# cocowy1/Cost-Volume-Aggregation-in-Stereo-Matching-Revisited

Hardware: AMD Instinct MI355X
Metric: cost-volumes/sec (fwd+bwd) at 544x960 D=192 (higher is better)
Workload: dtype f32

## Files before the change

### cost-volume-aggregation-in-stereo-matching-revisited_amd/csrc/conv3d_c1.hip

```cpp
#include "dca_common.h"
#include "dca_tiles.h"
#include "../../include/dca_hip.h"

namespace {
constexpr int TD = 4, TH = 8, TW = 32, CK = 4;
constexpr int ID = TD + 2, IH = TH + 2, IWP = 40;

struct C1Args {
  const float* x;
  const float* w;
  const float* dy;
  float* out;
  int N, C, D, H, W;
  int nTD, nTH, nTW, ntiles;
  int vec;
};

__device__ __forceinline__ void stage_tile(const float* __restrict__ src, float* lds, int n, int C, int c0, int nch,
                                           int D, int H, int W, int d0, int h0, int w0, int vec, int tid) {
  const int rows = nch * ID * IH;
  if (vec) {
    for (int it = tid; it < rows * 8; it += 256) {
      const int row = it >> 3, q = it & 7;
      const int c = row / (ID * IH), rem = row % (ID * IH), id = rem / IH, ih = rem % IH;
// ... 17 lines not shown
      const int row = it / 34, j = it % 34;
      const int c = row / (ID * IH), rem = row % (ID * IH), id = rem / IH, ih = rem % IH;
      const int ci = c0 + c, d = d0 - 1 + id, h = h0 - 1 + ih, wi = w0 - 1 + j;
      float v = 0.f;
      if (ci < C && (unsigned)d < (unsigned)D && (unsigned)h < (unsigned)H && (unsigned)wi < (unsigned)W)
        v = src[((((long)n * C + ci) * D + d) * H + h) * W + wi];
      lds[row * IWP + 3 + j] = v;
    }
  }
}

__device__ __forceinline__ void tile_coords(const C1Args& a, int tile, int& n, int& d0, int& h0, int& w0) {
  dca_tile_decode<TD, TH, TW>(tile, a.nTD, a.nTH, a.nTW, n, d0, h0, w0);
}

__global__ __launch_bounds__(256) void c1_bwd_data_kernel(C1Args a) {
  __shared__ __attribute__((aligned(16))) float dy_lds[ID * IH * IWP];
  extern __shared__ __attribute__((aligned(16))) float w_lds[];
  const int tid = threadIdx.x, wq = tid & 7, row = tid >> 3, dl = row >> 3, hl = row & 7;
  int n, d0, h0, w0;
  tile_coords(a, xcd_remap(blockIdx.x, gridDim.x), n, d0, h0, w0);
  stage_tile(a.dy, dy_lds, n, 1, 0, 1, a.D, a.H, a.W, d0, h0, w0, a.vec, tid);
  for (int i = tid; i < a.C * 27; i += 256) {
    const int c = i / 27, t = i % 27;
    w_lds[(c * 9 + t / 3) * 4 + t % 3] = a.w[c * 27 + 26 - t];
  }
  __syncthreads();
  float g[9][6];
#pragma unroll
  for (int r9 = 0; r9 < 9; ++r9) {
    const float* p = dy_lds + ((dl + r9 / 3) * IH + hl + r9 % 3) * IWP + 4 * wq;
    const float4 v = *(const float4*)(p + 4);
    g[r9][0] = p[3]; g[r9][1] = v.x; g[r9][2] = v.y; g[r9][3] = v.z; g[r9][4] = v.w; g[r9][5] = p[8];
  }
  const int d = d0 + dl, h = h0 + hl, w = w0 + 4 * wq;
  const bool ok = d < a.D && h < a.H && w < a.W;
  for (int c = 0; c < a.C; ++c) {
    float acc[4] = {0.f, 0.f, 0.f, 0.f};
#pragma unroll
    for (int r9 = 0; r9 < 9; ++r9) {
      const float4 wv = *(const float4*)(w_lds + (c * 9 + r9) * 4);
#pragma unroll
      for (int j = 0; j < 4; ++j)
        acc[j] = fmaf(wv.z, g[r9][j + 2], fmaf(wv.y, g[r9][j + 1], fmaf(wv.x, g[r9][j], acc[j])));
    }
    if (ok) {
      float* o = a.out + ((((long)n * a.C + c) * a.D + d) * a.H + h) * a.W + w;
      if (a.vec) {
        *(float4*)o = make_float4(acc[0], acc[1], acc[2], acc[3]);
      } else {
#pragma unroll
        for (int j = 0; j < 4; ++j)
          if (w + j < a.W) o[j] = acc[j];
      }
    }
  }
}

__global__ __launch_bounds__(256) void c1_gather_kernel(const float* __restrict__ T, float* __restrict__ y, int D, int H,
                                                        int W) {
  const long DHW = (long)D * H * W;
  const long n = blockIdx.y;
  const float* p = T + n * 27 * DHW;
  const long end = min(DHW, ((long)blockIdx.x + 1) * 1024);
  for (long idx = (long)blockIdx.x * 1024 + threadIdx.x; idx < end; idx += 256) {
    const int w = idx % W;
    const int t = (int)(idx / W);
    const int h = t % H, d = t / H;
// ... 55 lines not shown
      for (int j = 0; j < 4; ++j) v[j] = dca_bload1(dr, base + 4 * j, okr & (int)((unsigned)(w0 + j) < (unsigned)W));
    }
    *(float4*)(out + 4 * (long)q) = make_float4(v[0], v[1], v[2], v[3]);
  }
}

int fill_args(C1Args& a, int N, int C, int D, int H, int W, const void* p0, const void* p1, const void* p2) {
  a.N = N; a.C = C; a.D = D; a.H = H; a.W = W;
  a.nTD = cdiv(D, TD); a.nTH = cdiv(H, TH); a.nTW = cdiv(W, TW);
  const long nt = (long)N * a.nTD * a.nTH * a.nTW;
  if (nt >= (1L << 31)) return 1;
  a.ntiles = (int)nt;
  a.vec = (W % 4 == 0) && ((((uintptr_t)p0 | (uintptr_t)p1 | (uintptr_t)p2) & 15) == 0);
  return 0;
}
}

extern "C" int dca_conv3d_c1_bwd_data(const float* dy, const float* w, float* dx, int N, int C, int D, int H, int W,
                                      hipStream_t stream) {
  DCA_REQUIRE(dy && w && dx && N > 0 && C > 0 && C <= 256 && D > 0 && H > 0 && W > 0);
  C1Args a;
  a.x = nullptr; a.w = w; a.dy = dy; a.out = dx;
  DCA_REQUIRE(fill_args(a, N, C, D, H, W, dy, dx, nullptr) == 0);
  hipLaunchKernelGGL(c1_bwd_data_kernel, dim3(a.ntiles), dim3(256), (size_t)C * 36 * 4, stream, a);
  return dca_launch_status();
}

extern "C" int dca_conv3d_c1_gather(const float* T, float* y, int N, int D, int H, int W, hipStream_t stream) {
  DCA_REQUIRE(T && y && N > 0 && D > 0 && H > 0 && W > 0);
  DCA_REQUIRE(9L * D * H * W * 4 < 0x7ffffff0L && N <= 65535);
// ... 15 lines not shown
```

### cost-volume-aggregation-in-stereo-matching-revisited_amd/csrc/pointwise.hip

```cpp
#include "dca_frag.h"
#include "../../include/dca_hip.h"

__global__ __launch_bounds__(256) void bn_stats_kernel(const float* __restrict__ x, double* __restrict__ part, int N,
                                                       int C, long S, int nchunk, long chunk_len, int vec) {
  const int c = blockIdx.x, ch = blockIdx.y, tid = threadIdx.x;
  const long s0 = ch * chunk_len, s1 = min(S, s0 + chunk_len);
  const float K = x[(long)c * S];
  if (ch == 0 && tid == 0) part[(long)C * nchunk * 2 + c] = (double)K;
  float s = 0.f, ss = 0.f;
  for (int n = 0; n < N; ++n) {
    const float* p = x + ((long)n * C + c) * S;
    if (vec) {
      for (long i = s0 + 4 * tid; i < s1; i += 1024) {
        float4 v = *(const float4*)(p + i);
        v.x -= K; v.y -= K; v.z -= K; v.w -= K;
        s += (v.x + v.y) + (v.z + v.w);
        ss += (v.x * v.x + v.y * v.y) + (v.z * v.z + v.w * v.w);
      }
    } else {
      for (long i = s0 + tid; i < s1; i += 256) {
        const float v = p[i] - K;
        s += v;
        ss += v * v;
      }
// ... 96 lines not shown
  const float mean = (float)(kref + ms), var = (float)v;
  if (running_mean) {
    const double unb = n > 1.0 ? v * n / (n - 1.0) : v;
    running_mean[c] = (1.f - momentum) * running_mean[c] + momentum * mean;
    running_var[c] = (1.f - momentum) * running_var[c] + momentum * (float)unb;
  }
  const float invstd = 1.0f / sqrtf(var + eps);
  stats[c] = mean;
  stats[C + c] = invstd;
  stats[2 * C + c] = g * invstd;
  stats[3 * C + c] = b - mean * g * invstd;
  if (zexps) zexps[c] = ze;
}


__device__ __forceinline__ float bn_affine(float y, float sc, float sh) { return __fmaf_rn(y, sc, sh); }
__device__ __forceinline__ float bn_skip(float y, float sc, float sh) { return act_apply(bn_affine(y, sc, sh), 1.f); }
__device__ __forceinline__ void bn_bwd_acc(float g, float y, float mean, float invstd, float& a0, float& a1) {
#pragma clang fp contract(off)
  a0 += g;
  a1 += g * (y - mean) * invstd;
}

__global__ __launch_bounds__(256) void bn_apply_kernel(const float* __restrict__ y, const float* __restrict__ stats,
                                                       const float* __restrict__ res_pre, const float* __restrict__ res_post,
                                                       float* __restrict__ z, int N, int C, long S, long chunk_len,
                                                       float slope, int vec, unsigned* __restrict__ zmax,
                                                       unsigned* __restrict__ ymax) {
  const int c = blockIdx.y, ch = blockIdx.x, tid = threadIdx.x;
  const long s0 = ch * chunk_len, s1 = min(S, s0 + chunk_len);
  const float mean = stats[c], sc = stats[2 * C + c], sh = stats[3 * C + c];
  float am = 0.f, ym = 0.f;
  for (int n = N - 1; n >= 0; --n) {
    const long base = ((long)n * C + c) * S;
    if (vec) {
      for (long i = s0 + 4 * tid; i < s1; i += 1024) {
        float4 v = *(const float4*)(y + base + i);
// ... 9 lines not shown
      for (long i = s0 + tid; i < s1; i += 256) {
        const float yv = y[base + i];
        ym = fmaxf(ym, fabsf(yv - mean));
        float v = bn_affine(yv, sc, sh);
        if (res_pre) v += res_pre[base + i];
        v = act_apply(v, slope);
        if (res_post) v += res_post[base + i];
        z[base + i] = v;
        am = fmaxf(am, fabsf(v));
      }
    }
  }
  if (zmax) dca_cmax_put(am, zmax + (long)c * DCA_AMAX_CSLOTS + ch);
  if (ymax) dca_cmax_put(ym, ymax + (long)c * DCA_AMAX_CSLOTS + ch);
}

__device__ __forceinline__ void px2_split(float v, int e, unsigned short& h, unsigned short& l) {
  _Float16 hh, ll;
  x2_split(v, e, hh, ll);
  h = __builtin_bit_cast(unsigned short, hh);
  l = __builtin_bit_cast(unsigned short, ll);
}
typedef unsigned short u16x8 __attribute__((ext_vector_type(8)));

template <bool SKIP>
__global__ __launch_bounds__(256) void bn_apply_pack_kernel(const float* __restrict__ y, const float* __restrict__ stats,
                                                            const int* __restrict__ zexps, char* __restrict__ zp, int N,
                                                            int C, long S, long chunk_len, float slope,
                                                            unsigned* __restrict__ ymax, const float* __restrict__ res_pre,
                                                            const float* __restrict__ res_post, float* __restrict__ zf,
                                                            unsigned* __restrict__ zmax, const float* __restrict__ y_r,
                                                            const float* __restrict__ stats_r) {
  const int cg = blockIdx.y, ch = blockIdx.x, tid = threadIdx.x;
  const long s0 = ch * chunk_len, s1 = min(S, s0 + chunk_len);
  float mean[8], sc[8], sh[8], scr[8], shr[8], ym[8], zm[8];
  int ex[8];
#pragma unroll
  for (int j = 0; j < 8; ++j) {
// ... 910 lines not shown

extern "C" int dca_bn_backward_reduce(const float* dz, const float* y, const float* stats, double* part, float* dgb, int N,
                                      int C, long S, float slope, int training, hipStream_t stream) {
  DCA_REQUIRE(dz && y && stats && part && dgb && N > 0 && C > 0 && S > 0 && C <= 65535);
  int nchunk; long len;
  chunking(S, C, &nchunk, &len);
  const int vec = (S % 4 == 0) && ((((uintptr_t)dz | (uintptr_t)y) & 15) == 0);
  hipLaunchKernelGGL(bn_bwd_reduce_kernel, dim3(C, nchunk), dim3(256), 0, stream, dz, y, (const float*)nullptr, stats, part,
                     N, C, S, nchunk, len, slope, vec, (unsigned*)nullptr, (const float*)nullptr, (const float*)nullptr,
                     (double*)nullptr);
  hipLaunchKernelGGL(bn_bwd_finalize_kernel, dim3(C), dim3(64), 0, stream, part, nchunk, (double)N * (double)S, dgb, C,
                     stats, training, (const unsigned*)nullptr, (const unsigned*)nullptr, 0, (int*)nullptr);
  return dca_launch_status();
}

extern "C" int dca_bn_backward_pack(const float* dz, const float* y, const float* stats, double* part, float* dgb, void* dyp,
                                    int* dyexps, unsigned* gmax, const unsigned* ymax, int ymax_slots, int N, int C, long S,
                                    float slope, int training, hipStream_t stream) {
  DCA_REQUIRE(dz && y && stats && part && dgb && dyp && dyexps && gmax && N > 0 && C > 0 && C % 8 == 0 && S > 0 && C <= 65535);
  DCA_REQUIRE((ymax == nullptr || (ymax_slots > 0 && ymax_slots <= DCA_AMAX_CSLOTS)) && ((((uintptr_t)dyp) & 15) == 0));
  int nchunk; long len;
  chunking(S, C, &nchunk, &len);
  const uintptr_t al = (uintptr_t)dz | (uintptr_t)y;
  const int vec = (S % 4 == 0) && ((al & 15) == 0);
  hipLaunchKernelGGL(bn_bwd_reduce_kernel, dim3(C, nchunk), dim3(256), 0, stream, dz, y, (const float*)nullptr, stats, part,
                     N, C, S, nchunk, len, slope, vec, gmax, (const float*)nullptr, (const float*)nullptr, (double*)nullptr);
  hipLaunchKernelGGL(bn_bwd_finalize_kernel, dim3(C), dim3(64), 0, stream, part, nchunk, (double)N * (double)S, dgb, C,
                     stats, training, (const unsigned*)gmax, ymax, ymax_slots, dyexps);
  int pchunk; long plen;
  chunking(S, C / 8, &pchunk, &plen);
// ... 66 lines not shown
```

### cost-volume-aggregation-in-stereo-matching-revisited_amd/models/augment/cva.py

```python
import torch
import torch.nn as nn

from .._bootstrap import ensure as _ensure
from ..submodule import ConvBn3d, ConvBnReLU3d, conv3d_plain, convbn_3d
from .semantic_level import SemanticLevelContext

ops = _ensure().ops


class _DeconvBn3d(nn.Sequential):

    def __init__(self, cin, cout):
        super().__init__(nn.ConvTranspose3d(cin, cout, 3, padding=1, output_padding=1, stride=2, bias=False),
                         nn.BatchNorm3d(cout))

    def forward(self, x, slope=1.0, res_pre=None, res_post=None, pack_out=False):
        return ops.convbn3d(x, self[0], self[1], slope, res_pre, res_post, pack_out=pack_out)


class Multi_Aggregation(nn.Module):

    def __init__(self, in_channels):
        super().__init__()
        self.conv1 = ConvBnReLU3d(in_channels, in_channels * 2, 3, 2, 1)
# ... 15 lines not shown
                         nn.ReLU(inplace=True))

    def forward(self, x):
        return self[1](ops.avg_pool3d_k3s2p1(x), slope=0.0)


class _Classify(nn.Sequential):

    def __init__(self, c):
        super().__init__(ConvBn3d(c, c, 3, 1, 1), nn.ReLU(inplace=True),
                         nn.Conv3d(c, 1, kernel_size=3, padding=1, stride=1, bias=False))

    def forward(self, x, alias=False):
        if alias:
            h, xa = self[0](x, slope=0.0, alias=True)
            return conv3d_plain(h, self[2]), xa
        h = self[0](x, slope=0.0)
        if h.dtype != torch.float32:
            return ops.conv3d_c1_lp(h, self[2].weight)
        return conv3d_plain(h, self[2])


class cva(nn.Module):

    def __init__(self, max_disp, in_channel, downsample=True):
        super().__init__()
        self.max_disp = max_disp
        self.channel = in_channel
        if downsample:
            self.downsample = _Downsample()
        self.slc_net = SemanticLevelContext(feats_channels=self.channel, transform_channels=self.channel,
                                            concat_input=True)
        self.classify = _Classify(self.channel)
        self.fuse = nn.Sequential(ConvBn3d(64, 32, 1, 1, 0))
        self.cost_agg = Multi_Aggregation(self.channel)
# ... 40 lines not shown
```

### cost-volume-aggregation-in-stereo-matching-revisited_amd/models/submodule.py

```python
import torch
import torch.nn as nn
import torch.nn.functional as F

from ._bootstrap import ensure as _ensure

ops = _ensure().ops


def disparity_regression(x, maxdisp):
    assert len(x.shape) == 4
    assert x.shape[1] == maxdisp
    return ops.regression(x)


def build_concat_volume(refimg_fea, targetimg_fea, maxdisp):
    return ops.concat_volume(refimg_fea, targetimg_fea, maxdisp)


def groupwise_correlation(fea1, fea2, num_groups):
    B, C, H, W = fea1.shape
    assert C % num_groups == 0
    cost = ops.gwc_volume(fea1, fea2, 1, num_groups)[:, :, 0]
    assert cost.shape == (B, num_groups, H, W)
    return cost
# ... 17 lines not shown
        assert (kernel_size, pad) in ((3, 1), (1, 0)) and stride in (1, 2)

    def forward(self, x, slope=1.0, res_pre=None, res_post=None, x2=None, alias=False, pack_out=False):
        return ops.convbn3d(x, self[0], self[1], slope, res_pre, res_post, x2, alias, pack_out)


class ConvBnReLU3d(nn.Sequential):

    def __init__(self, in_channels, out_channels, kernel_size, stride, pad):
        super().__init__(ConvBn3d(in_channels, out_channels, kernel_size, stride, pad), nn.ReLU(inplace=True))

    def forward(self, x):
        return self[0](x, slope=0.0)


def conv3d_plain(x, conv):
    return ops.conv3d(x, conv.weight, conv.stride[0], False)


def convbn(in_channels, out_channels, kernel_size, stride, pad, dilation):
    return nn.Sequential(nn.Conv2d(in_channels, out_channels, kernel_size=kernel_size, stride=stride,
                                   padding=dilation if dilation > 1 else pad, dilation=dilation, bias=False),
                         nn.BatchNorm2d(out_channels))


class BasicBlock(nn.Module):
    expansion = 1

    def __init__(self, inplanes, planes, stride, downsample, pad, dilation):
        super().__init__()
        self.conv1 = nn.Sequential(convbn(inplanes, planes, 3, stride, pad, dilation), nn.ReLU(inplace=True))
        self.conv2 = convbn(planes, planes, 3, 1, pad, dilation)
# ... 99 lines not shown
```

### cost-volume-aggregation-in-stereo-matching-revisited_amd/ops.py

```python
from __future__ import annotations

import ctypes
import os
import threading

import torch

from ._call import _C, _L, _chk, _ptr, _raw_device, _raw_stream, _req, _req_no_grad, _stream, _vp


def _opt(t, name):
    return None if t is None else _req(t, name)


class _GwcVolume(torch.autograd.Function):
    @staticmethod
    def forward(ctx, ref, tgt, maxdisp, num_groups):
        ref, tgt = _req(ref, "build_gwc_volume"), _req(tgt, "build_gwc_volume")
        B, C, H, W = ref.shape
        vol = torch.empty((B, num_groups, maxdisp, H, W), device=ref.device, dtype=torch.float32)
        with torch.cuda.device_of(ref):
            _chk(_L().dca_gwc_volume_fwd(_ptr(ref), _ptr(tgt), _ptr(vol), B, C, H, W, maxdisp, num_groups, _stream()),
                 "dca_gwc_volume_fwd")
        ctx.save_for_backward(ref, tgt)
# ... 208 lines not shown

def _round_up(a, m):
    return (a + m - 1) // m * m


_CONV_MODE = os.environ.get("DCA_CONV", "x2")
CONV_X3 = _CONV_MODE != "fp32"
CONV_X2 = _CONV_MODE == "x2"
WGRAD_S2_X2 = os.environ.get("DCA_WGRAD_S2", "x2") != "fp32"
DECONV_X3 = os.environ.get("DCA_DECONV", "x3") != "fp32"
C1_WGRAD_FUSED = os.environ.get("DCA_C1_WGRAD", "fused") != "expand"
CONV_S2_X2 = os.environ.get("DCA_CONV_S2", "x2") != "fp32"
BN_FUSE = os.environ.get("DCA_BN_FUSE", "1") != "0"
C1_BWD_FUSE = os.environ.get("DCA_C1_BWD", "fused") != "split"
SKIP_FOLD = os.environ.get("DCA_SKIP_FOLD", "1") != "0"
_X3_MIN_WORKGROUPS = 1


AMAX_STATS = {"tagged": 0, "computed": 0, "packed": 0}
CSLOTS = _C["DCA_AMAX_CSLOTS"]
AMAX_EMIT = os.environ.get("DCA_AMAX_EMIT", "1") != "0"
PACK = os.environ.get("DCA_PACK", "1") != "0"


def _cslots(C, device):
    if not AMAX_EMIT:
        return None
    return torch.empty((C * CSLOTS,), device=device, dtype=torch.int32)


# ... 163 lines not shown
    y, stats, dgb, slope, training = tag
    if y.shape != dz.shape or y.shape[0] != x.shape[0] or y.shape[2:] != x.shape[2:]:
        raise RuntimeError("conv3d.backward: the BatchNorm's gradient does not belong to this convolution")
    N, C1 = x.shape[0], x.shape[1]
    C2 = 0 if x2 is None else x2.shape[1]
    S = x[0, 0].numel()
    lib = _L()
    part = torch.empty((lib.dca_conv1_bwd_fused_workspace(N, S, int(x2 is not None)),), device=x.device, dtype=torch.float32)
    gx = torch.empty_like(x)
    gx2 = None if x2 is None else torch.empty_like(x2)
    gw = torch.empty_like(weight)
    _chk(lib.dca_conv1_bwd_fused(_ptr(dz), _ptr(y), _ptr(stats), _ptr(dgb), float(slope), int(training), _ptr(x), _ptr(x2),
                                 _ptr(weight), _ptr(part), _ptr(gx), _ptr(gx2), _ptr(gw), C1 + C2, 1, N, C1, C2,
                                 weight.shape[0], S, _stream()), "dca_conv1_bwd_fused")
    return gx, gx2, gw


class _SkipBn:
    __slots__ = ("y", "part", "bn", "into")

    def __init__(self, y, part, bn, into):
        self.y, self.part, self.bn, self.into = y, part, bn, into


def _skip_fold_route(x, conv_b, bn_b, slope_b, bn_out):
    if not (SKIP_FOLD and PACK and CONV_X2 and bn_out is not None and torch.is_grad_enabled() and _lp_dtype() is None):
        return "apply"
    C = bn_b.num_features
    if not (bn_b.training and bn_out.training) or bn_out.num_features != C or C % 8 or float(slope_b) != 1.0:
        return "apply"
# ... 215 lines not shown
             "dca_conv3d_wgrad_x3")
    elif family == "s2x2":
        xex, yex = _exps_of(x), _exps_of(dy)
        part = workspace(lib.dca_conv3d_wgrad_s2_x2_workspace(N, Cx, Cy, Di, Hi, Wi))
        _chk(lib.dca_conv3d_wgrad_s2_x2(_ptr(x), _ptr(xex), _ptr(dy), _ptr(yex), _ptr(part), dst, N, Cx, Cy, Di, Hi, Wi,
                                        s_cy, s_cx, _stream()), "dca_conv3d_wgrad_s2_x2")
    else:
        part = workspace(lib.dca_conv3d_wgrad_workspace(N, Cx, Cy, Do, Ho, Wo, ksize, stride))
        _chk(lib.dca_conv3d_wgrad(_ptr(x), _ptr(dy), _ptr(part), dst, N, Cx, Cy, Di, Hi, Wi, Do, Ho, Wo, ksize, stride,
                                  s_cy, s_cx, _stream()), "dca_conv3d_wgrad")


class _Conv3dC1(torch.autograd.Function):

    @staticmethod
    def forward(ctx, x, weight):
        x, weight = _req(x, "conv3d"), _req(weight, "conv3d.weight")
        N, C, D, H, W = x.shape
        with torch.cuda.device_of(x):
            T = _conv_sliced(x, None, weight, C, 27, 1, 1, 0, 1, 1, False)
            y = torch.empty((N, 1, D, H, W), device=x.device, dtype=torch.float32)
            _chk(_L().dca_conv3d_c1_gather(_ptr(T), _ptr(y), N, D, H, W, _stream()), "dca_conv3d_c1_gather")
        ctx.save_for_backward(x, weight)
        return y

    @staticmethod
    def backward(ctx, dy):
        x, weight = ctx.saved_tensors
        dy = _req(dy, "conv3d.backward")
        N, C, D, H, W = x.shape
        gx = gw = None
        lib = _L()
        with torch.cuda.device_of(x):
            if ctx.needs_input_grad[0]:
                gx = torch.empty_like(x)
                _chk(lib.dca_conv3d_c1_bwd_data(_ptr(dy), _ptr(weight), _ptr(gx), N, C, D, H, W, _stream()),
                     "dca_conv3d_c1_bwd_data")
            if ctx.needs_input_grad[1]:
                gw = torch.empty_like(weight)
                if (C1_WGRAD_FUSED and W % 4 == 0 and x.data_ptr() % 16 == 0 and dy.data_ptr() % 16 == 0
                        and x.numel() * 4 < 0x7ffffff0):
                    nws = lib.dca_conv3d_wgrad_workspace(N, C, 27, D, H, W, 1, 1)
                    part = torch.empty((nws,), device=x.device, dtype=torch.float32)
                    _chk(lib.dca_conv3d_c1_wgrad(_ptr(x), _ptr(dy), _ptr(part), _ptr(gw), N, C, D, H, W, _stream()),
                         "dca_conv3d_c1_wgrad")
                else:
                    G = torch.empty((N, 27, D, H, W), device=x.device, dtype=torch.float32)
                    _chk(lib.dca_conv3d_c1_expand(_ptr(dy), _ptr(G), N, D, H, W, _stream()), "dca_conv3d_c1_expand")
                    _wgrad(x, G, gw, 0, C, 27, 1, 1, 1, 27)
        return gx, gw


class _Conv3d(torch.autograd.Function):

    @staticmethod
    def forward(ctx, x, x2, weight, stride, transposed, want_stats=False, alias=False, packed_dy=False, lazy_dy=False):
        x, weight = _req(x, "conv3d", packed_ok=True), _req(weight, "conv3d.weight")
        x2 = _opt(x2, "conv3d.x2")
        if _is_packed(x) and alias:
            raise RuntimeError("conv3d: alias output of a packed px2 operand")
        ctx.save_for_backward(x, x2, weight)
        ctx.meta = (stride, transposed)
        ctx.alias = bool(alias)
        ctx.set_materialize_grads(False)
        ctx.x_px2 = getattr(x, "_dca_px2", None)
# ... 140 lines not shown
          and conv_b.kernel_size[0] == 1 and conv_b.weight.shape[0] in (32, 64) and x.dtype == torch.float32
          and not isinstance(conv_a, torch.nn.ConvTranspose3d) and all(d % 2 == 0 for d in x.shape[2:]))
    if not ok:
        return convbn3d(x, conv_a, bn_a, slope_a, pack_out=pack_a), convbn3d(x, conv_b, bn_b, slope_b)
    stats = bool(BN_FUSE and bn_a.training and bn_b.training)
    fold = _skip_fold_route(x, conv_b, bn_b, slope_b, skip_into) == "fold"
    lazy = fold or _c1_bwd_route(x, None, conv_b.weight) == "fused"
    ya, pa, yb, pb = _ConvPair.apply(x, conv_a.weight, conv_b.weight, stats, lazy)
    za = bn_act(ya, bn_a, slope_a, stats_part=pa if pa.numel() else None, pack_out=pack_a)
    if fold:
        return za, _SkipBn(yb, pb if pb.numel() else None, bn_b, skip_into)
    zb = bn_act(yb, bn_b, slope_b, stats_part=pb if pb.numel() else None, lazy_dy=lazy)
    return za, zb


def conv3d(x, weight, stride=1, transposed=False, x2=None):
    if _k3s1(weight, stride, transposed, x2, head=True) and weight.shape[1] in (32, 64):
        return _Conv3dC1.apply(x, weight)
    return _Conv3d.apply(x, x2, weight, int(stride), bool(transposed))


def conv3d_fused_inference(x, weight, stride, transposed, scale, shift, slope, res_pre=None, res_post=None, x2=None):
    x, weight = _req(x, "conv3d"), _req(weight, "conv3d.weight")
    with torch.cuda.device_of(x):
        return _conv_forward_impl(x, _opt(x2, "x2"), weight, int(stride), bool(transposed), _opt(scale, "scale"),
                                  _opt(shift, "shift"), slope, _opt(res_pre, "res_pre"), _opt(res_post, "res_post"),
                                  emit_amax=CONV_X2 and AMAX_EMIT)


def bn_stats_vector(y, gamma, beta, running_mean, running_var, training, momentum, eps, part=None, zexps=None,
                    rpre=None, rpost=None):
    rps, rpn = rpre if rpre is not None else (None, 0)
# ... 65 lines not shown
                _tag_px2(zp, zexps)
                if pack_z == 2:
                    _tag_twin(z, zp)
            else:
                _chk(lib.dca_bn_apply(_ptr(y), _ptr(stats), _ptr(res_pre), _ptr(res_post), _ptr(z), N, C, S, float(slope),
                                      _ptr(zmax), _ptr(ymax), _stream()), "dca_bn_apply")
                ymax_slots = lib.dca_bn_num_chunks(C, S)
        ctx.save_for_backward(y, stats, res_pre if slope != 1.0 else None, ymax)
        ctx.meta = (training, slope, res_pre is not None, res_post is not None, pack_dy, ymax_slots)
        return z if pack_z == 1 else _tag_cmax(z, zmax, ymax_slots)

    @staticmethod
    def backward(ctx, dz):
        y, stats, res_pre, ymax = ctx.saved_tensors
        training, slope, has_pre, has_post, pack_dy, ymax_slots = ctx.meta
        dz = _req(dz, "batch_norm.backward")
        N, C = y.shape[0], y.shape[1]
        S = y[0, 0].numel()
        lib = _L()
        with torch.cuda.device_of(y):
            nchunk = lib.dca_bn_num_chunks(C, S)
            part = torch.empty((C * nchunk * 2,), device=y.device, dtype=torch.float64)
            dgb = torch.empty((4 * C,), device=y.device, dtype=torch.float32)
            g_out = None
            if ctx.lazy_dy:
                _chk(lib.dca_bn_backward_reduce(_ptr(dz), _ptr(y), _ptr(stats), _ptr(part), _ptr(dgb), N, C, S, float(slope),
                                                int(training), _stream()), "dca_bn_backward_reduce")
                dy = dz.view_as(dz)
                dy._dca_lazy = (y, stats, dgb, slope, training)
            elif pack_dy:
# ... 6 lines not shown
                _tag_px2(dy, dyexps)
            else:
                dy = torch.empty_like(y)
                want_g = has_pre and slope != 1.0 and ctx.needs_input_grad[9]
                g_out = torch.empty_like(y) if want_g else None
                dm = _cslots(C, y.device) if CONV_X2 else None
                _chk(lib.dca_bn_backward(_ptr(dz), _ptr(y), _ptr(res_pre), _ptr(stats), _ptr(part), _ptr(dgb), _ptr(dy),
                                         _ptr(g_out), N, C, S, float(slope), int(training), _ptr(dm), _stream()),
                     "dca_bn_backward")
                _tag_cmax(dy, dm, nchunk)
        g_pre = None
        if has_pre and ctx.needs_input_grad[9]:
            g_pre = g_out if g_out is not None else dz
        g_post = dz if (has_post and ctx.needs_input_grad[10]) else None
        return dy, dgb[:C], dgb[C:2 * C], None, None, None, None, None, None, g_pre, g_post, None, None, None, None, None


class _BnSkipAct(torch.autograd.Function):

    @staticmethod
    def forward(ctx, y, gamma, beta, running_mean, running_var, momentum, eps, part, y_r, gamma_r, beta_r, running_mean_r,
                running_var_r, momentum_r, eps_r, part_r, slope, res_post, zmax):
        y, y_r = _req(y, "batch_norm"), _req(y_r, "batch_norm.skip")
        res_post = _opt(res_post, "res_post")
        if y_r.shape != y.shape:
            raise RuntimeError("batch_norm: the skip branch does not have the output's shape")
        N, C = y.shape[0], y.shape[1]
        S = y[0, 0].numel()
        lib = _L()
        with torch.cuda.device_of(y):
# ... 736 lines not shown
```

### include/dca_hip.h

```cpp
#ifndef DCA_HIP_H
#define DCA_HIP_H

#include <hip/hip_runtime_api.h>

#ifdef __cplusplus
extern "C" {
#endif

#define DCA_ABI_VERSION 21
int dca_abi_version(void);

#define DCA_BF16 1
#define DCA_FP16 2

int dca_gwc_volume_fwd(const float* ref, const float* tgt, float* vol, int B, int C, int H, int W, int maxdisp,
                       int num_groups, hipStream_t stream);
int dca_gwc_volume_bwd(const float* gvol, const float* ref, const float* tgt, float* gref, float* gtgt, int B, int C,
                       int H, int W, int maxdisp, int num_groups, hipStream_t stream);
long dca_gwc_volume_bwd_rows(int B, int C, int H, int W, int maxdisp, int num_groups);
int dca_concat_volume_fwd(const float* ref, const float* tgt, float* vol, int B, int C, int H, int W, int maxdisp,
                          hipStream_t stream);
int dca_concat_volume_bwd(const float* gvol, float* gref, float* gtgt, int B, int C, int H, int W, int maxdisp,
                          hipStream_t stream);

// ... 105 lines not shown
                    int* zexps, const unsigned* rpre_slots, int rpre_n, const unsigned* rpost_slots, int rpost_n, int C,
                    hipStream_t stream);
int dca_bn_apply(const float* y, const float* stats, const float* res_pre, const float* res_post, float* z, int N,
                 int C, long S, float slope, unsigned* zmax, unsigned* ymax, hipStream_t stream);
int dca_bn_apply_pack(const float* y, const float* stats, const int* zexps, void* zp, int N, int C, long S, float slope,
                      unsigned* ymax, const float* res_pre, const float* res_post, float* zf, unsigned* zmax,
                      hipStream_t stream);
int dca_bn_backward(const float* dz, const float* y, const float* res_pre, const float* stats, double* part,
                    float* dgb, float* dy, float* g_out, int N, int C, long S, float slope, int training,
                    unsigned* dmax, hipStream_t stream);
int dca_bn_backward_reduce(const float* dz, const float* y, const float* stats, double* part, float* dgb, int N, int C,
                           long S, float slope, int training, hipStream_t stream);
int dca_bn_backward_pack(const float* dz, const float* y, const float* stats, double* part, float* dgb, void* dyp,
                         int* dyexps, unsigned* gmax, const unsigned* ymax, int ymax_slots, int N, int C, long S,
                         float slope, int training, hipStream_t stream);
int dca_bn_skip_max(const float* y_r, const float* stats_r, int N, int C, long S, unsigned* slots, hipStream_t stream);
int dca_bn_apply_pack_skip(const float* y, const float* stats, const int* zexps, void* zp, int N, int C, long S, float slope,
                           unsigned* ymax, const float* y_r, const float* stats_r, const float* res_post, float* zf,
                           unsigned* zmax, hipStream_t stream);
int dca_bn_backward_skip(const float* dz, const float* y, const float* y_r, const float* stats, const float* stats_r,
                         double* part, double* part_r, float* dgb, float* dgb_r, float* dy, float* g_out, int N, int C,
                         long S, float slope, int training, unsigned* dmax, hipStream_t stream);

int dca_avgpool3d_fwd(const float* x, float* y, long NC, int Di, int Hi, int Wi, hipStream_t stream);
int dca_avgpool3d_bwd(const float* gy, float* gx, const float* res, const float* res2, long NC, int Di, int Hi, int Wi,
                     hipStream_t stream);

int dca_trilinear_fwd(const float* x, float* y, long NC, int Di, int Hi, int Wi, int scale, hipStream_t stream);
int dca_trilinear_bwd(const float* gy, float* gx, long NC, int Di, int Hi, int Wi, int scale, hipStream_t stream);

// ... 209 lines not shown
```

Measured before the change: 42.49.

## Fuse logit-head conv backward-data into preceding BatchNorm backward pack

When the single-output-channel head conv is the only reader of a BN+ReLU output, its backward no longer writes the full 32-channel input gradient. Instead it hands off the 1-channel dlogit and the weights, and the BN backward recomputes the 3x3x3 transposed conv on the fly in both its reduce pass and its apply/pack pass. This removes the write and re-read of a large fp32 gradient tensor. In exchange the conv arithmetic is done twice, and the path relies on autograd tagging of an expanded tensor, which is fragile.

```diff
diff --git a/cost-volume-aggregation-in-stereo-matching-revisited_amd/csrc/bn_math.h b/cost-volume-aggregation-in-stereo-matching-revisited_amd/csrc/bn_math.h
--- /dev/null
+++ b/cost-volume-aggregation-in-stereo-matching-revisited_amd/csrc/bn_math.h
@@ -0,0 +1,22 @@
+#pragma once
+#include "dca_frag.h"
+
+__device__ __forceinline__ float bn_affine(float y, float sc, float sh) { return __fmaf_rn(y, sc, sh); }
+__device__ __forceinline__ void bn_bwd_acc(float g, float y, float mean, float invstd, float& a0, float& a1) {
+#pragma clang fp contract(off)
+  a0 += g;
+  a1 += g * (y - mean) * invstd;
+}
+
+__device__ __forceinline__ void px2_split(float v, int e, unsigned short& h, unsigned short& l) {
+  _Float16 hh, ll;
+  x2_split(v, e, hh, ll);
+  h = __builtin_bit_cast(unsigned short, hh);
+  l = __builtin_bit_cast(unsigned short, ll);
+}
+typedef unsigned short u16x8 __attribute__((ext_vector_type(8)));
+
+void dca_internal_bn_chunking(long S, int C, int* nchunk, long* chunk_len);
+int dca_internal_bn_bwd_finalize(const double* part, int nchunk, double count, float* dgb, int C, const float* stats,
+                                 int training, const unsigned* gmax, const unsigned* ymax, int ymax_slots, int* dyexps,
+                                 hipStream_t stream);
diff --git a/cost-volume-aggregation-in-stereo-matching-revisited_amd/csrc/conv3d_c1.hip b/cost-volume-aggregation-in-stereo-matching-revisited_amd/csrc/conv3d_c1.hip
--- a/cost-volume-aggregation-in-stereo-matching-revisited_amd/csrc/conv3d_c1.hip
+++ b/cost-volume-aggregation-in-stereo-matching-revisited_amd/csrc/conv3d_c1.hip
@@ -1,5 +1,6 @@
 #include "dca_common.h"
 #include "dca_tiles.h"
+#include "bn_math.h"
 #include "../../include/dca_hip.h"
 
 namespace {
@@ -55,6 +56,39 @@
   dca_tile_decode<TD, TH, TW>(tile, a.nTD, a.nTH, a.nTW, n, d0, h0, w0);
 }
 
+__device__ __forceinline__ void c1_stage_weights(const float* __restrict__ w, float* w_lds, int C, int tid) {
+  for (int i = tid; i < C * 27; i += 256) {
+    const int c = i / 27, t = i % 27;
+    w_lds[(c * 9 + t / 3) * 4 + t % 3] = w[c * 27 + 26 - t];
+  }
+}
+__device__ __forceinline__ void c1_window(const float* dy_lds, int dl, int hl, int wq, float (&g)[9][6]) {
+#pragma unroll
+  for (int r9 = 0; r9 < 9; ++r9) {
+    const float* p = dy_lds + ((dl + r9 / 3) * IH + hl + r9 % 3) * IWP + 4 * wq;
+    const float4 v = *(const float4*)(p + 4);
+    g[r9][0] = p[3]; g[r9][1] = v.x; g[r9][2] = v.y; g[r9][3] = v.z; g[r9][4] = v.w; g[r9][5] = p[8];
+  }
+}
+__device__ __forceinline__ void c1_dx4_row(const float (&g)[6], float wx, float wy, float wz, float (&acc)[4]) {
+#pragma unroll
+  for (int j = 0; j < 4; ++j)
+    acc[j] = fmaf(wz, g[j + 2], fmaf(wy, g[j + 1], fmaf(wx, g[j], acc[j])));
+}
+__device__ __forceinline__ void c1_dx4(const float* w_lds, int c, const float (&g)[9][6], float (&acc)[4]) {
+  acc[0] = acc[1] = acc[2] = acc[3] = 0.f;
+#pragma unroll
+  for (int r9 = 0; r9 < 9; ++r9) {
+    const float4 wv = *(const float4*)(w_lds + (c * 9 + r9) * 4);
+    c1_dx4_row(g[r9], wv.x, wv.y, wv.z, acc);
+  }
+}
+__device__ __forceinline__ void c1_dx4_s(const float* __restrict__ wc, const float (&g)[9][6], float (&acc)[4]) {
+  acc[0] = acc[1] = acc[2] = acc[3] = 0.f;
+#pragma unroll
+  for (int r9 = 0; r9 < 9; ++r9) c1_dx4_row(g[r9], wc[26 - 3 * r9], wc[25 - 3 * r9], wc[24 - 3 * r9], acc);
+}
+
 __global__ __launch_bounds__(256) void c1_bwd_data_kernel(C1Args a) {
   __shared__ __attribute__((aligned(16))) float dy_lds[ID * IH * IWP];
   extern __shared__ __attribute__((aligned(16))) float w_lds[];
@@ -62,29 +96,15 @@
   int n, d0, h0, w0;
   tile_coords(a, xcd_remap(blockIdx.x, gridDim.x), n, d0, h0, w0);
   stage_tile(a.dy, dy_lds, n, 1, 0, 1, a.D, a.H, a.W, d0, h0, w0, a.vec, tid);
-  for (int i = tid; i < a.C * 27; i += 256) {
-    const int c = i / 27, t = i % 27;
-    w_lds[(c * 9 + t / 3) * 4 + t % 3] = a.w[c * 27 + 26 - t];
-  }
+  c1_stage_weights(a.w, w_lds, a.C, tid);
   __syncthreads();
   float g[9][6];
-#pragma unroll
-  for (int r9 = 0; r9 < 9; ++r9) {
-    const float* p = dy_lds + ((dl + r9 / 3) * IH + hl + r9 % 3) * IWP + 4 * wq;
-    const float4 v = *(const float4*)(p + 4);
-    g[r9][0] = p[3]; g[r9][1] = v.x; g[r9][2] = v.y; g[r9][3] = v.z; g[r9][4] = v.w; g[r9][5] = p[8];
-  }
+  c1_window(dy_lds, dl, hl, wq, g);
   const int d = d0 + dl, h = h0 + hl, w = w0 + 4 * wq;
   const bool ok = d < a.D && h < a.H && w < a.W;
   for (int c = 0; c < a.C; ++c) {
-    float acc[4] = {0.f, 0.f, 0.f, 0.f};
-#pragma unroll
-    for (int r9 = 0; r9 < 9; ++r9) {
-      const float4 wv = *(const float4*)(w_lds + (c * 9 + r9) * 4);
-#pragma unroll
-      for (int j = 0; j < 4; ++j)
-        acc[j] = fmaf(wv.z, g[r9][j + 2], fmaf(wv.y, g[r9][j + 1], fmaf(wv.x, g[r9][j], acc[j])));
-    }
+    float acc[4];
+    c1_dx4(w_lds, c, g, acc);
     if (ok) {
       float* o = a.out + ((((long)n * a.C + c) * a.D + d) * a.H + h) * a.W + w;
       if (a.vec) {
@@ -93,6 +113,160 @@
 #pragma unroll
         for (int j = 0; j < 4; ++j)
           if (w + j < a.W) o[j] = acc[j];
+      }
+    }
+  }
+}
+
+constexpr int BC = 32;
+
+struct C1BnArgs {
+  const float* dlogit;
+  const float* y;
+  const float* stats;
+  const float* dgb;
+  const int* dyexps;
+  double* part;
+  unsigned* gmax;
+  int N, D, H, W;
+  int nTD, nTH, nTW, ntiles;
+  float slope;
+  int training;
+};
+
+__device__ __forceinline__ int c1_per_tile(int tid) {
+  asm volatile("" : "+v"(tid));
+  return tid;
+}
+
+constexpr int RCG = 4;
+__global__ __launch_bounds__(256, 2) void c1_bn_bwd_reduce_kernel(C1BnArgs a, const float* __restrict__ wt, int nchunk,
+                                                                  int chunk_len) {
+  const int ch = blockIdx.x, cg = blockIdx.y, tid = threadIdx.x;
+  const int HW = a.H * a.W, S = a.D * HW;
+  const int s0 = ch * chunk_len, s1 = min(S, s0 + chunk_len);
+  float mean[RCG], invstd[RCG], sc[RCG], sh[RCG], a0[RCG], a1[RCG], gm[RCG];
+#pragma unroll
+  for (int j = 0; j < RCG; ++j) {
+    const int c = cg * RCG + j;
+    mean[j] = a.stats[c]; invstd[j] = a.stats[BC + c]; sc[j] = a.stats[2 * BC + c]; sh[j] = a.stats[3 * BC + c];
+    a0[j] = a1[j] = gm[j] = 0.f;
+  }
+  for (int n = a.N - 1; n >= 0; --n) {
+    const __amdgpu_buffer_rsrc_t rd = dca_rsrc(a.dlogit + (long)n * S, (long)S * 4);
+    const __amdgpu_buffer_rsrc_t ry = dca_rsrc(a.y + (long)n * BC * S, (long)BC * S * 4);
+    for (int i = s0 + 4 * tid; i < s1; i += 1024) {
+      const int d = i / HW, r = i - d * HW, h = r / a.W, w = r - h * a.W;
+      float g[9][6];
+#pragma unroll
+      for (int r9 = 0; r9 < 9; ++r9) {
+        const int dd = d + r9 / 3 - 1, hh = h + r9 % 3 - 1;
+        const int okr = (int)((unsigned)dd < (unsigned)a.D) & (int)((unsigned)hh < (unsigned)a.H);
+        const int base = ((dd * a.H + hh) * a.W + w) * 4;
+        const float4 v = dca_bload4(rd, base, okr);
+        g[r9][0] = dca_bload1(rd, base - 4, okr & (int)(w > 0));
+        g[r9][1] = v.x; g[r9][2] = v.y; g[r9][3] = v.z; g[r9][4] = v.w;
+        g[r9][5] = dca_bload1(rd, base + 16, okr & (int)(w + 4 < a.W));
+      }
+      float4 yv[RCG];
+#pragma unroll
+      for (int j = 0; j < RCG; ++j) yv[j] = dca_bload4(ry, ((cg * RCG + j) * S + i) * 4, 1);
+#pragma unroll
+      for (int j = 0; j < RCG; ++j) {
+        float dh[4];
+        c1_dx4_s(wt + (cg * RCG + j) * 27, g, dh);
+        const float ys[4] = {yv[j].x, yv[j].y, yv[j].z, yv[j].w};
+#pragma unroll
+        for (int e = 0; e < 4; ++e) {
+          const float u = bn_affine(ys[e], sc[j], sh[j]);
+          const float gg = dh[e] * (u > 0.f ? 1.f : a.slope);
+          bn_bwd_acc(gg, ys[e], mean[j], invstd[j], a0[j], a1[j]);
+          gm[j] = fmaxf(gm[j], fabsf(gg));
+        }
+      }
+    }
+  }
+  __shared__ double red[8];
+#pragma unroll
+  for (int j = 0; j < RCG; ++j) {
+    const int c = cg * RCG + j;
+    const double d0 = wave_sum_d((double)a0[j]), d1 = wave_sum_d((double)a1[j]);
+    __syncthreads();
+    if ((tid & 63) == 0) { red[(tid >> 6) * 2] = d0; red[(tid >> 6) * 2 + 1] = d1; }
+    __syncthreads();
+    if (tid == 0) {
+      a.part[((long)c * nchunk + ch) * 2 + 0] = red[0] + red[2] + red[4] + red[6];
+      a.part[((long)c * nchunk + ch) * 2 + 1] = red[1] + red[3] + red[5] + red[7];
+    }
+    dca_cmax_put(gm[j], a.gmax + (long)c * DCA_AMAX_CSLOTS + ch);
+  }
+}
+
+
+__global__ __launch_bounds__(256, 4) void c1_bn_bwd_apply_pack_kernel(C1BnArgs a, const float* __restrict__ wt,
+                                                                      char* __restrict__ dyp) {
+  __shared__ __attribute__((aligned(16))) float dy_lds[ID * IH * IWP];
+  __shared__ __attribute__((aligned(16))) float k_lds[BC * 8];
+  const int tid = threadIdx.x, wq = tid & 7, row = tid >> 3, dl = row >> 3, hl = row & 7;
+  const int S = a.D * a.H * a.W;
+  if (tid < BC) {
+    const int c = tid;
+    float* k = k_lds + c * 8;
+    k[0] = a.stats[c]; k[1] = a.stats[2 * BC + c]; k[2] = a.stats[3 * BC + c];
+    k[3] = a.training ? dca_coherent_loadf(a.dgb + 2 * BC + c) : 0.f;
+    k[4] = a.training ? dca_coherent_loadf(a.dgb + 3 * BC + c) * a.stats[BC + c] : 0.f;
+    k[5] = __int_as_float(dca_coherent_loadi(a.dyexps + c));
+  }
+  const long tb = px2_term_bytes(BC, S);
+  for (int tile = blockIdx.x; tile < a.ntiles; tile += (int)gridDim.x) {
+    int n, d0, h0, w0;
+    dca_tile_decode<TD, TH, TW>(tile, a.nTD, a.nTH, a.nTW, n, d0, h0, w0);
+    __syncthreads();
+    stage_tile(a.dlogit, dy_lds, n, 1, 0, 1, a.D, a.H, a.W, d0, h0, w0, 1, c1_per_tile(tid));
+    __syncthreads();
+    float g[9][6];
+    c1_window(dy_lds, dl, hl, wq, g);
+    const int d = d0 + dl, h = h0 + hl, w = w0 + 4 * wq;
+    const int ok = (int)(d < a.D) & (int)(h < a.H) & (int)(w < a.W);
+    const __amdgpu_buffer_rsrc_t ry = dca_rsrc(a.y + (long)n * BC * S, (long)BC * S * 4);
+    const int vox = (d * a.H + h) * a.W + w;
+    char* ob = dyp + (long)n * 2 * tb + (long)vox * 16;
+#pragma unroll 1
+    for (int cg = 0; cg < BC / 8; ++cg) {
+      float4 yv[8];
+#pragma unroll
+      for (int j = 0; j < 8; ++j) yv[j] = dca_bload4(ry, ((cg * 8 + j) * S + vox) * 4, ok);
+      unsigned hv[4][4], lv[4][4];
+#pragma unroll
+      for (int j = 0; j < 8; ++j) {
+        const int c = cg * 8 + j;
+        float dh[4];
+        c1_dx4_s(wt + c * 27, g, dh);
+        const float4 ka = *(const float4*)(k_lds + c * 8), kb = *(const float4*)(k_lds + c * 8 + 4);
+        const float mean = ka.x, sc = ka.y, sh = ka.z, k1 = ka.w, k2 = kb.x;
+        const int ex = __float_as_int(kb.y);
+        const float ys[4] = {yv[j].x, yv[j].y, yv[j].z, yv[j].w};
+#pragma unroll
+        for (int e = 0; e < 4; ++e) {
+          const float u = bn_affine(ys[e], sc, sh);
+          const float gg = dh[e] * (u > 0.f ? 1.f : a.slope);
+          const float o = (gg - k1 - (ys[e] - mean) * k2) * sc;
+          unsigned short hh, ll;
+          px2_split(o, ex, hh, ll);
+          if (j % 2 == 0) {
+            hv[e][j / 2] = hh; lv[e][j / 2] = ll;
+          } else {
+            hv[e][j / 2] |= (unsigned)hh << 16; lv[e][j / 2] |= (unsigned)ll << 16;
+          }
+        }
+      }
+      if (ok) {
+        char* p = ob + (long)cg * S * 16;
+#pragma unroll
+        for (int e = 0; e < 4; ++e) {
+          *(uint4*)(p + e * 16) = make_uint4(hv[e][0], hv[e][1], hv[e][2], hv[e][3]);
+          *(uint4*)(p + tb + e * 16) = make_uint4(lv[e][0], lv[e][1], lv[e][2], lv[e][3]);
+        }
       }
     }
   }
@@ -178,6 +352,49 @@
   a.vec = (W % 4 == 0) && ((((uintptr_t)p0 | (uintptr_t)p1 | (uintptr_t)p2) & 15) == 0);
   return 0;
 }
+
+struct C1BnGeom {
+  DcaTileGrid t;
+  int nchunk, nwg_apply;
+  long chunk_len;
+};
+C1BnGeom c1_bn_geometry(int N, int D, int H, int W) {
+  C1BnGeom g;
+  g.t = dca_tile_grid<TD, TH, TW>(N, D, H, W);
+  dca_internal_bn_chunking((long)D * H * W, BC, &g.nchunk, &g.chunk_len);
+  const long cap = 4L * dca_num_cus(), half = g.t.tiles > 1 ? (g.t.tiles + 1) / 2 : 1;
+  g.nwg_apply = (int)(half < cap ? half : cap);
+  return g;
+}
+}
+
+extern "C" int dca_bn_backward_pack_c1_chunks(int N, int D, int H, int W) { return c1_bn_geometry(N, D, H, W).nchunk; }
+extern "C" int dca_bn_backward_pack_c1_grid(int N, int D, int H, int W) { return c1_bn_geometry(N, D, H, W).nwg_apply; }
+
+extern "C" int dca_bn_backward_pack_c1(const float* dlogit, const float* w_head, const float* y, const float* stats,
+                                       double* part, float* dgb, void* dyp, int* dyexps, unsigned* gmax, const unsigned* ymax,
+                                       int ymax_slots, int N, int C, int D, int H, int W, float slope, int training,
+                                       hipStream_t stream) {
+  DCA_REQUIRE(dlogit && w_head && y && stats && part && dgb && dyp && dyexps && gmax);
+  DCA_REQUIRE(N > 0 && C == BC && D > 0 && H > 0 && W > 0 && W % 4 == 0);
+  DCA_REQUIRE((long)C * D * H * W * 4 < 0x7ffffff0L);
+  DCA_REQUIRE(((((uintptr_t)dlogit) | ((uintptr_t)y) | ((uintptr_t)dyp)) & 15) == 0);
+  DCA_REQUIRE(ymax == nullptr || (ymax_slots > 0 && ymax_slots <= DCA_AMAX_CSLOTS));
+  const C1BnGeom g = c1_bn_geometry(N, D, H, W);
+  DCA_REQUIRE(g.t.fits() && g.nchunk <= DCA_AMAX_CSLOTS);
+  C1BnArgs a;
+  a.dlogit = dlogit; a.y = y; a.stats = stats; a.dgb = dgb; a.dyexps = dyexps;
+  a.part = part; a.gmax = gmax;
+  a.N = N; a.D = D; a.H = H; a.W = W;
+  a.nTD = g.t.nTD; a.nTH = g.t.nTH; a.nTW = g.t.nTW; a.ntiles = (int)g.t.tiles;
+  a.slope = slope; a.training = training;
+  hipLaunchKernelGGL(c1_bn_bwd_reduce_kernel, dim3(g.nchunk, BC / RCG), dim3(256), 0, stream, a, w_head, g.nchunk,
+                     (int)g.chunk_len);
+  const int rc = dca_internal_bn_bwd_finalize(part, g.nchunk, (double)N * (double)D * H * W, dgb, C, stats, training, gmax, ymax,
+                                              ymax_slots, dyexps, stream);
+  if (rc) return rc;
+  hipLaunchKernelGGL(c1_bn_bwd_apply_pack_kernel, dim3(g.nwg_apply), dim3(256), 0, stream, a, w_head, (char*)dyp);
+  return dca_launch_status();
 }
 
 extern "C" int dca_conv3d_c1_bwd_data(const float* dy, const float* w, float* dx, int N, int C, int D, int H, int W,
diff --git a/cost-volume-aggregation-in-stereo-matching-revisited_amd/csrc/pointwise.hip b/cost-volume-aggregation-in-stereo-matching-revisited_amd/csrc/pointwise.hip
--- a/cost-volume-aggregation-in-stereo-matching-revisited_amd/csrc/pointwise.hip
+++ b/cost-volume-aggregation-in-stereo-matching-revisited_amd/csrc/pointwise.hip
@@ -1,4 +1,4 @@
-#include "dca_frag.h"
+#include "bn_math.h"
 #include "../../include/dca_hip.h"
 
 __global__ __launch_bounds__(256) void bn_stats_kernel(const float* __restrict__ x, double* __restrict__ part, int N,
@@ -134,13 +134,7 @@
 }
 
 
-__device__ __forceinline__ float bn_affine(float y, float sc, float sh) { return __fmaf_rn(y, sc, sh); }
 __device__ __forceinline__ float bn_skip(float y, float sc, float sh) { return act_apply(bn_affine(y, sc, sh), 1.f); }
-__device__ __forceinline__ void bn_bwd_acc(float g, float y, float mean, float invstd, float& a0, float& a1) {
-#pragma clang fp contract(off)
-  a0 += g;
-  a1 += g * (y - mean) * invstd;
-}
 
 __global__ __launch_bounds__(256) void bn_apply_kernel(const float* __restrict__ y, const float* __restrict__ stats,
                                                        const float* __restrict__ res_pre, const float* __restrict__ res_post,
@@ -180,14 +174,6 @@
   if (zmax) dca_cmax_put(am, zmax + (long)c * DCA_AMAX_CSLOTS + ch);
   if (ymax) dca_cmax_put(ym, ymax + (long)c * DCA_AMAX_CSLOTS + ch);
 }
-
-__device__ __forceinline__ void px2_split(float v, int e, unsigned short& h, unsigned short& l) {
-  _Float16 hh, ll;
-  x2_split(v, e, hh, ll);
-  h = __builtin_bit_cast(unsigned short, hh);
-  l = __builtin_bit_cast(unsigned short, ll);
-}
-typedef unsigned short u16x8 __attribute__((ext_vector_type(8)));
 
 template <bool SKIP>
 __global__ __launch_bounds__(256) void bn_apply_pack_kernel(const float* __restrict__ y, const float* __restrict__ stats,
@@ -1128,6 +1114,16 @@
   return dca_launch_status();
 }
 
+void dca_internal_bn_chunking(long S, int C, int* nchunk, long* chunk_len) { chunking(S, C, nchunk, chunk_len); }
+
+int dca_internal_bn_bwd_finalize(const double* part, int nchunk, double count, float* dgb, int C, const float* stats,
+                                 int training, const unsigned* gmax, const unsigned* ymax, int ymax_slots, int* dyexps,
+                                 hipStream_t stream) {
+  hipLaunchKernelGGL(bn_bwd_finalize_kernel, dim3(C), dim3(64), 0, stream, part, nchunk, count, dgb, C, stats, training, gmax,
+                     ymax, ymax_slots, dyexps);
+  return dca_launch_status();
+}
+
 extern "C" int dca_bn_backward_pack(const float* dz, const float* y, const float* stats, double* part, float* dgb, void* dyp,
                                     int* dyexps, unsigned* gmax, const unsigned* ymax, int ymax_slots, int N, int C, long S,
                                     float slope, int training, hipStream_t stream) {
diff --git a/cost-volume-aggregation-in-stereo-matching-revisited_amd/models/augment/cva.py b/cost-volume-aggregation-in-stereo-matching-revisited_amd/models/augment/cva.py
--- a/cost-volume-aggregation-in-stereo-matching-revisited_amd/models/augment/cva.py
+++ b/cost-volume-aggregation-in-stereo-matching-revisited_amd/models/augment/cva.py
@@ -53,11 +53,11 @@
     def forward(self, x, alias=False):
         if alias:
             h, xa = self[0](x, slope=0.0, alias=True)
-            return conv3d_plain(h, self[2]), xa
+            return conv3d_plain(h, self[2], sole_reader=True), xa
         h = self[0](x, slope=0.0)
         if h.dtype != torch.float32:
             return ops.conv3d_c1_lp(h, self[2].weight)
-        return conv3d_plain(h, self[2])
+        return conv3d_plain(h, self[2], sole_reader=True)
 
 
 class cva(nn.Module):
diff --git a/cost-volume-aggregation-in-stereo-matching-revisited_amd/models/submodule.py b/cost-volume-aggregation-in-stereo-matching-revisited_amd/models/submodule.py
--- a/cost-volume-aggregation-in-stereo-matching-revisited_amd/models/submodule.py
+++ b/cost-volume-aggregation-in-stereo-matching-revisited_amd/models/submodule.py
@@ -55,8 +55,8 @@
         return self[0](x, slope=0.0)
 
 
-def conv3d_plain(x, conv):
-    return ops.conv3d(x, conv.weight, conv.stride[0], False)
+def conv3d_plain(x, conv, sole_reader=False):
+    return ops.conv3d(x, conv.weight, conv.stride[0], False, sole_reader=sole_reader)
 
 
 def convbn(in_channels, out_channels, kernel_size, stride, pad, dilation):
diff --git a/cost-volume-aggregation-in-stereo-matching-revisited_amd/ops.py b/cost-volume-aggregation-in-stereo-matching-revisited_amd/ops.py
--- a/cost-volume-aggregation-in-stereo-matching-revisited_amd/ops.py
+++ b/cost-volume-aggregation-in-stereo-matching-revisited_amd/ops.py
@@ -246,6 +246,7 @@
 BN_FUSE = os.environ.get("DCA_BN_FUSE", "1") != "0"
 C1_BWD_FUSE = os.environ.get("DCA_C1_BWD", "fused") != "split"
 SKIP_FOLD = os.environ.get("DCA_SKIP_FOLD", "1") != "0"
+C1_HEAD_BWD = os.environ.get("DCA_C1_HEAD_BWD", "fused") != "split"
 _X3_MIN_WORKGROUPS = 1
 
 
@@ -439,6 +440,24 @@
                                  _ptr(weight), _ptr(part), _ptr(gx), _ptr(gx2), _ptr(gw), C1 + C2, 1, N, C1, C2,
                                  weight.shape[0], S, _stream()), "dca_conv1_bwd_fused")
     return gx, gx2, gw
+
+
+def _c1_head_bwd_route(h, weight, sole_reader):
+    if not (C1_HEAD_BWD and sole_reader and torch.is_grad_enabled()):
+        return "split"
+    node = h.grad_fn
+    if not isinstance(node, _BnAct._backward_cls) or getattr(node, "meta", None) is None:
+        return "split"
+    training, slope, has_pre, has_post, pack_dy, _ = node.meta
+    if not (training and pack_dy and float(slope) == 0.0) or has_pre or has_post:
+        return "split"
+    if tuple(weight.shape) != (1, 32, 3, 3, 3) or h.dim() != 5 or h.shape[1] != 32 or h.shape[-1] % 4:
+        return "split"
+    if not all(t.is_cuda and t.dtype == torch.float32 and t.requires_grad for t in (h, weight)):
+        return "split"
+    if _is_packed(h) or h.data_ptr() % 16 or not h.is_contiguous() or h[0].numel() * 4 >= 0x7ffffff0:
+        return "split"
+    return "fused"
 
 
 class _SkipBn:
@@ -684,8 +703,9 @@
 class _Conv3dC1(torch.autograd.Function):
 
     @staticmethod
-    def forward(ctx, x, weight):
+    def forward(ctx, x, weight, head_fused=False):
         x, weight = _req(x, "conv3d"), _req(weight, "conv3d.weight")
+        ctx.head_fused = bool(head_fused)
         N, C, D, H, W = x.shape
         with torch.cuda.device_of(x):
             T = _conv_sliced(x, None, weight, C, 27, 1, 1, 0, 1, 1, False)
@@ -702,7 +722,10 @@
         gx = gw = None
         lib = _L()
         with torch.cuda.device_of(x):
-            if ctx.needs_input_grad[0]:
+            if ctx.head_fused:
+                gx = dy.expand(N, C, D, H, W)
+                gx._dca_head = (dy, weight)
+            elif ctx.needs_input_grad[0]:
                 gx = torch.empty_like(x)
                 _chk(lib.dca_conv3d_c1_bwd_data(_ptr(dy), _ptr(weight), _ptr(gx), N, C, D, H, W, _stream()),
                      "dca_conv3d_c1_bwd_data")
@@ -718,7 +741,7 @@
                     G = torch.empty((N, 27, D, H, W), device=x.device, dtype=torch.float32)
                     _chk(lib.dca_conv3d_c1_expand(_ptr(dy), _ptr(G), N, D, H, W, _stream()), "dca_conv3d_c1_expand")
                     _wgrad(x, G, gw, 0, C, 27, 1, 1, 1, 27)
-        return gx, gw
+        return gx, gw, None
 
 
 class _Conv3d(torch.autograd.Function):
@@ -889,8 +912,11 @@
     return za, zb
 
 
-def conv3d(x, weight, stride=1, transposed=False, x2=None):
+def conv3d(x, weight, stride=1, transposed=False, x2=None, sole_reader=False):
     if _k3s1(weight, stride, transposed, x2, head=True) and weight.shape[1] in (32, 64):
+        if _c1_head_bwd_route(x, weight, sole_reader) == "fused":
+            x.grad_fn.head_fused = True
+            return _Conv3dC1.apply(x, weight, True)
         return _Conv3dC1.apply(x, weight)
     return _Conv3d.apply(x, x2, weight, int(stride), bool(transposed))
 
@@ -986,6 +1012,8 @@
     def backward(ctx, dz):
         y, stats, res_pre, ymax = ctx.saved_tensors
         training, slope, has_pre, has_post, pack_dy, ymax_slots = ctx.meta
+        if getattr(ctx, "head_fused", False):
+            return _BnAct._backward_head(ctx, dz)
         dz = _req(dz, "batch_norm.backward")
         N, C = y.shape[0], y.shape[1]
         S = y[0, 0].numel()
@@ -1022,6 +1050,33 @@
             g_pre = g_out if g_out is not None else dz
         g_post = dz if (has_post and ctx.needs_input_grad[10]) else None
         return dy, dgb[:C], dgb[C:2 * C], None, None, None, None, None, None, g_pre, g_post, None, None, None, None, None
+
+    @staticmethod
+    def _backward_head(ctx, dz):
+        y, stats, _, ymax = ctx.saved_tensors
+        training, slope, _, _, _, ymax_slots = ctx.meta
+        tag = getattr(dz, "_dca_head", None)
+        if tag is None:
+            raise RuntimeError("batch_norm.backward: expected the hand-off of the logit head behind this BatchNorm (its output "
+                               "has another reader besides the head, or the tag was lost on the way through autograd)")
+        dlogit, w_head = tag
+        N, C, D, H, W = y.shape
+        if dlogit.shape != (N, 1, D, H, W) or dz.shape != y.shape:
+            raise RuntimeError("batch_norm.backward: the head's hand-off does not belong to this BatchNorm")
+        lib = _L()
+        with torch.cuda.device_of(y):
+            nchunk = lib.dca_bn_backward_pack_c1_chunks(N, D, H, W)
+            part = torch.empty((C * nchunk * 2,), device=y.device, dtype=torch.float64)
+            dgb = torch.empty((4 * C,), device=y.device, dtype=torch.float32)
+            dyexps = torch.empty((C,), device=y.device, dtype=torch.int32)
+            gmax = torch.empty((C * CSLOTS,), device=y.device, dtype=torch.int32)
+            dy = torch.empty_like(y)
+            _chk(lib.dca_bn_backward_pack_c1(_ptr(dlogit), _ptr(w_head), _ptr(y), _ptr(stats), _ptr(part), _ptr(dgb), _ptr(dy),
+                                             _ptr(dyexps), _ptr(gmax), _ptr(ymax), ymax_slots if ymax is not None else 0,
+                                             N, C, D, H, W, float(slope), int(training), _stream()),
+                 "dca_bn_backward_pack_c1")
+            _tag_px2(dy, dyexps)
+        return dy, dgb[:C], dgb[C:2 * C], None, None, None, None, None, None, None, None, None, None, None, None, None
 
 
 class _BnSkipAct(torch.autograd.Function):
diff --git a/include/dca_hip.h b/include/dca_hip.h
--- a/include/dca_hip.h
+++ b/include/dca_hip.h
@@ -143,6 +143,11 @@
 int dca_bn_backward_pack(const float* dz, const float* y, const float* stats, double* part, float* dgb, void* dyp,
                          int* dyexps, unsigned* gmax, const unsigned* ymax, int ymax_slots, int N, int C, long S,
                          float slope, int training, hipStream_t stream);
+int dca_bn_backward_pack_c1_chunks(int N, int D, int H, int W);
+int dca_bn_backward_pack_c1_grid(int N, int D, int H, int W);
+int dca_bn_backward_pack_c1(const float* dlogit, const float* w_head, const float* y, const float* stats, double* part,
+                            float* dgb, void* dyp, int* dyexps, unsigned* gmax, const unsigned* ymax, int ymax_slots, int N,
+                            int C, int D, int H, int W, float slope, int training, hipStream_t stream);
 int dca_bn_skip_max(const float* y_r, const float* stats_r, int N, int C, long S, unsigned* slots, hipStream_t stream);
 int dca_bn_apply_pack_skip(const float* y, const float* stats, const int* zexps, void* zp, int N, int C, long S, float slope,
                            unsigned* ymax, const float* y_r, const float* stats_r, const float* res_post, float* zf,
```

Result: faster. 42.98, median of 6 (+1.2%).
